# mims-harvard/ProCyon

Measured on AMD Instinct MI355X. Metric: phenotype-gen tokens/sec (ProCyon-Full greedy generation, end to end), higher is better.
Workload: dtype bf16; 1 GPU; configs[1]: ProCyon-Full (ESM2-650M + Llama-3-8B geometry=full) bf16 batch=1, 1024-residue protein, 512-token prompt, 256-token greedy generation; parallelism=single GPU

## Files before the change

include/pcy.h:

```cpp
#ifndef PCY_H
#define PCY_H
#include <stddef.h>
#include <stdint.h>

#ifdef __cplusplus
extern "C" {
#endif

#define PCY_ABI_VERSION 13

typedef struct pcy_ctx pcy_ctx;

enum { PCY_EPI_STORE = 0, PCY_EPI_RESID = 1, PCY_EPI_GELU_ERF = 2, PCY_EPI_GELU_ESM = 3, PCY_EPI_SWIGLU = 4 };
enum { PCY_POOL_MEAN = 0, PCY_POOL_MEAN_CORRECTED = 1, PCY_POOL_MAX = 2 };

int pcy_abi_version(void);
unsigned long long pcy_debug_dispatch_count(int kind);
unsigned long long pcy_debug_extend_grouped_count(void);
const char* pcy_last_error(void);
int pcy_ctx_create(int device_id, void* stream, pcy_ctx** out);
void pcy_ctx_destroy(pcy_ctx* ctx);
int pcy_ctx_sync(pcy_ctx* ctx);
int pcy_timer_start(pcy_ctx* ctx);
int pcy_timer_stop(pcy_ctx* ctx, float* ms_out);
// ... 169 lines not shown
  const int32_t* forced;
  int32_t* counters;
  int32_t* last;
  int32_t cap, W;
  int32_t ngram_max, ngram_min;
} pcy_look_state;
int pcy_look_draft(pcy_ctx*, const pcy_llama_desc*, const pcy_look_state*, const pcy_gen_state*, void* embeds_out);
int pcy_look_verify(pcy_ctx*, const pcy_llama_desc*, const pcy_look_state*, const pcy_gen_state*, const void* logits);
unsigned long long pcy_debug_look_count(int which);
int pcy_attn_window(pcy_ctx*, void* qkv, int ld, const pcy_kv_cache* kv, int layer, void* o, int ldo, const int32_t* pos, const void* cos_t,
                    const void* sin_t, int W, int H, int Hkv, int dh);
int pcy_attn_window_chunk(void);
int pcy_llama_decode_window(pcy_ctx*, const pcy_llama_desc*, const pcy_kv_cache*, const pcy_gen_state*, const void* embeds, int W,
                            void* logits_out);
unsigned long long pcy_debug_decode_window_count(void);
int pcy_llama_greedy(pcy_ctx*, const pcy_llama_desc*, const pcy_kv_cache*, const pcy_gen_state*, int B, int n_steps,
                     int use_graph);
int pcy_sample_pick(pcy_ctx*, const pcy_llama_desc*, const pcy_kv_cache*, const pcy_gen_state*, int B, int advance_pos,
                    float temperature, float nucleus_prob, const float* uniforms, void* probs_out);
int pcy_llama_sample(pcy_ctx*, const pcy_llama_desc*, const pcy_kv_cache*, const pcy_gen_state*, int B, int n_steps,
                     float temperature, float nucleus_prob, const float* uniforms);
typedef struct {
  int32_t* out; int32_t max_len;
  float* cur; float* cur_new;
  int32_t* next_tok;
  int32_t* src;
  int32_t* anc;
  uint8_t* has_eos;
  int32_t* blk_eos; int32_t* ticket;
  int32_t* pos; int32_t* step; int32_t* done;
// ... 40 lines not shown
```

procyon_amd/_lib.py:

```python
from __future__ import annotations

import ctypes as C
import os

_HERE = os.path.dirname(os.path.abspath(__file__))
LIB_PATH = os.environ.get("PCY_LIB") or os.path.join(_HERE, "libpcy.so")

EPI_STORE, EPI_RESID, EPI_GELU_ERF, EPI_GELU_ESM, EPI_SWIGLU = range(5)
POOL_MEAN, POOL_MEAN_CORRECTED, POOL_MAX = range(3)
ABI_VERSION = 13
(DISPATCH_GEMM_128, DISPATCH_GEMM_64, DISPATCH_GEMM_BIG, DISPATCH_GEMM_BIG_PERSIST, DISPATCH_GEMM_SPLITK, DISPATCH_GEMM_FP8, DISPATCH_ATTN_FAST,
 DISPATCH_DEC_STEP_GQA, DISPATCH_GEMM_MID, DISPATCH_ESM_GRAPH, DISPATCH_DEC_STEP_MHA, DISPATCH_DEC_LAYER, DISPATCH_DEC_STEP_NB, DISPATCH_DEC_STEP_MB,
 DISPATCH_DEC_LOOP_STREAM, DISPATCH_DEC_LOOP_MFMA, DISPATCH_SHARED_PREFIX, DISPATCH_XENT, DISPATCH_EXTEND,
 DISPATCH_EXTEND_PACKED) = range(20)
DISPATCH_DECODE = dict(step_gqa=DISPATCH_DEC_STEP_GQA, step_mha=DISPATCH_DEC_STEP_MHA, layer=DISPATCH_DEC_LAYER, step_nb=DISPATCH_DEC_STEP_NB,
                       step_mb=DISPATCH_DEC_STEP_MB, loop_stream=DISPATCH_DEC_LOOP_STREAM, loop_mfma=DISPATCH_DEC_LOOP_MFMA)
ATTN_ROUTE_DH32, ATTN_ROUTE_DH64, ATTN_ROUTE_LDS128_1, ATTN_ROUTE_LDS128_2 = range(4)

vp = C.c_void_p
i32 = C.c_int32
ci = C.c_int


class MlpDesc(C.Structure):
# ... 119 lines not shown
    "pcy_attn_decode_shared": (ci, [vp, vp, ci, C.POINTER(KvCache), ci, vp, ci, vp, vp, vp, vp, ci, ci, ci, ci]),
    "pcy_llama_decode_gemm_mq": (ci, [vp, C.POINTER(LlamaDesc), C.POINTER(KvCache), C.POINTER(GenState), ci]),
    "pcy_debug_attn_mq_count": (C.c_ulonglong, []),
    "pcy_gemv_w8": (ci, [vp, vp, vp, vp, ci, vp, vp, ci, vp, C.c_float, ci, ci, ci, ci, ci]),
    "pcy_llama_decode_w8": (ci, [vp, C.POINTER(LlamaDesc), C.POINTER(LlamaLayerFp8), C.POINTER(KvCache), C.POINTER(GenState), ci]),
    "pcy_llama_greedy_w8": (ci, [vp, C.POINTER(LlamaDesc), C.POINTER(LlamaLayerFp8), C.POINTER(KvCache), C.POINTER(GenState), ci, ci, ci]),
    "pcy_debug_decode_w8_count": (C.c_ulonglong, []),
    "pcy_greedy_pick": (ci, [vp, C.POINTER(LlamaDesc), C.POINTER(KvCache), C.POINTER(GenState), ci, ci]),
    "pcy_look_draft": (ci, [vp, C.POINTER(LlamaDesc), C.POINTER(LookState), C.POINTER(GenState), vp]),
    "pcy_look_verify": (ci, [vp, C.POINTER(LlamaDesc), C.POINTER(LookState), C.POINTER(GenState), vp]),
    "pcy_debug_look_count": (C.c_ulonglong, [ci]),
    "pcy_attn_window": (ci, [vp, vp, ci, C.POINTER(KvCache), ci, vp, ci, vp, vp, vp, ci, ci, ci, ci]),
    "pcy_attn_window_chunk": (ci, []),
    "pcy_llama_decode_window": (ci, [vp, C.POINTER(LlamaDesc), C.POINTER(KvCache), C.POINTER(GenState), vp, ci, vp]),
    "pcy_debug_decode_window_count": (C.c_ulonglong, []),
    "pcy_llama_greedy": (ci, [vp, C.POINTER(LlamaDesc), C.POINTER(KvCache), C.POINTER(GenState), ci, ci, ci]),
    "pcy_sample_pick": (ci, [vp, C.POINTER(LlamaDesc), C.POINTER(KvCache), C.POINTER(GenState), ci, ci, C.c_float, C.c_float, vp, vp]),
    "pcy_llama_sample": (ci, [vp, C.POINTER(LlamaDesc), C.POINTER(KvCache), C.POINTER(GenState), ci, ci, C.c_float, C.c_float, vp]),
    "pcy_beam_step": (ci, [vp, vp, ci, ci, ci, ci, C.c_float, C.POINTER(BeamState)]),
    "pcy_kv_reorder": (ci, [vp, C.POINTER(LlamaDesc), C.POINTER(KvCache), vp, ci, ci]),
    "pcy_kv_reorder_range": (ci, [vp, C.POINTER(LlamaDesc), C.POINTER(KvCache), vp, ci, ci, ci]),
    "pcy_llama_beam_steps": (ci, [vp, C.POINTER(LlamaDesc), C.POINTER(KvCache), C.POINTER(GenState), ci, ci, ci, C.c_float, C.POINTER(BeamState), vp, ci, ci]),
}

_lib = None


class PcyError(RuntimeError):
    pass

# ... 25 lines not shown
```

procyon_amd/csrc/pcy_elem.hip:

```cpp
#include "pcy_internal.h"
#include "pcy_pick.h"

namespace {

constexpr int NT = 256;

__global__ __launch_bounds__(NT) void rmsnorm_kernel(const bf16_t* __restrict__ x, const bf16_t* __restrict__ w,
                                                     bf16_t* __restrict__ y, int d, float eps, int cast) {
  __shared__ float red[NT / 64];
  const bf16_t* xr = x + (size_t)blockIdx.x * d;
  bf16_t* yr = y + (size_t)blockIdx.x * d;
  float ss = 0.f;
  for (int k = threadIdx.x * 8; k < d; k += NT * 8) {
    const uint4 v = *reinterpret_cast<const uint4*>(xr + k);
    const uint32_t u[4] = {v.x, v.y, v.z, v.w};
#pragma unroll
    for (int j = 0; j < 4; ++j) { float a = lo_bf(u[j]), b = hi_bf(u[j]); ss += a * a + b * b; }
  }
  ss = block_sum<NT>(ss, red);
  const float rstd = rsqrtf(ss / (float)d + eps);
  for (int k = threadIdx.x * 8; k < d; k += NT * 8) {
    const uint4 v = *reinterpret_cast<const uint4*>(xr + k);
    const uint4 g = *reinterpret_cast<const uint4*>(w + k);
    const uint32_t u[4] = {v.x, v.y, v.z, v.w}, gg[4] = {g.x, g.y, g.z, g.w};
// ... 375 lines not shown
  const int w = threadIdx.x >> 6;
  if ((threadIdx.x & 63) == 0) { redv[w] = best; redi[w] = bi; }
  __syncthreads();
  best = redv[0]; bi = redi[0];
  for (int i = 1; i < PICK_NT / 64; ++i)
    if (redv[i] > best || (redv[i] == best && redi[i] < bi)) { best = redv[i]; bi = redi[i]; }
  float se = 0.f;
  for (int i = lo + threadIdx.x; i < hi; i += PICK_NT) se += expf(bf2f(lg[i]) - best);
  se = block_sum<PICK_NT>(se, red);
  if (threadIdx.x == 0) part[b * PICK_NB + c] = PickPartial{best, bi, best > -INFINITY ? se : 0.f, 0};
}

__global__ __launch_bounds__(256) void pick_stage2_kernel(const bf16_t* __restrict__ logits, int V, const PickPartial* __restrict__ part,
                                                          int32_t* __restrict__ next_tok, int32_t* __restrict__ tokens_out, int max_steps,
                                                          float* __restrict__ logprob, int32_t* __restrict__ step_dev, int32_t* __restrict__ pos_dev,
                                                          int advance_pos, int B) {
  const int l = threadIdx.x & 63;
  const int step = *step_dev;
  for (int b = threadIdx.x >> 6; b < B; b += 4) {
    float best, se;
    int bi;
    pick_merge_row(part[b * PICK_NB + l], best, bi, se);
    if (l == 0) {
      const float lsm = pick_logprob(logits + (size_t)b * V, bi, best, se);
      logprob[b] += lsm;
      next_tok[b] = bi;
      tokens_out[(size_t)b * max_steps + step] = bi;
    }
  }
  __syncthreads();
  if (threadIdx.x == 0) { if (advance_pos) *pos_dev += 1; *step_dev = step + 1; }
}

constexpr int SMP_NT = 1024;

__global__ __launch_bounds__(PICK_NT) void sample_stage1_kernel(const bf16_t* __restrict__ logits, int V, float temperature,
                                                                float4* __restrict__ part) {
  __shared__ float red[PICK_NT / 64];
  const int b = blockIdx.y, c = blockIdx.x;
  const int chunk = (V + PICK_NB - 1) / PICK_NB;
  const int lo = c * chunk, hi = (lo + chunk) < V ? (lo + chunk) : V;
  const bf16_t* lg = logits + (size_t)b * V;
  const bool scaled = temperature != 1.0f;
  float mr = -INFINITY, ms = -INFINITY;
  for (int i = lo + threadIdx.x; i < hi; i += PICK_NT) {
    const float v = bf2f(lg[i]);
// ... 852 lines not shown
  hipLaunchKernelGGL(transpose_v_kernel, dim3((maxpad + 63) / 64, nh * dh / 64, nseq), dim3(NT), 0, s, buf, ld, vcol0, dh, cu, vt_cu, vt, vt_total);
}
size_t pcy_pool_ws_bytes(int nprot, int d) { return (size_t)nprot * POOL_CH * d * 8; }
void pcy_launch_pool(hipStream_t s, const bf16_t* h, int d, const int32_t* seg, const int32_t* rng, int nprot, int mode, bf16_t* out,
                     void* ws) {
  if (nprot <= 0) return;
  float* wsum = reinterpret_cast<float*>(ws);
  int* wcnt = reinterpret_cast<int*>(wsum + (size_t)nprot * POOL_CH * d);
  hipLaunchKernelGGL(pool_partial_kernel, dim3(nprot, (d + 511) / 512, POOL_CH), dim3(NT), 0, s, h, d, seg, rng, mode, wsum, wcnt);
  hipLaunchKernelGGL(pool_finish_kernel, dim3(nprot, (d + NT - 1) / NT), dim3(NT), 0, s, wsum, wcnt, d, mode, out);
}
void pcy_launch_pick_stage1(hipStream_t s, const bf16_t* logits, int rows, int V, void* partials) {
  if (rows > 0) hipLaunchKernelGGL(pick_stage1_kernel, dim3(PICK_NB, rows), dim3(PICK_NT), 0, s, logits, V, reinterpret_cast<PickPartial*>(partials));
}
void pcy_launch_greedy_pick(hipStream_t s, const bf16_t* logits, int B, int V, int32_t* next_tok, int32_t* tokens_out,
                            int max_steps, float* logprob, int32_t* pos_dev, int32_t* step_dev, int advance_pos, void* partials) {
  hipLaunchKernelGGL(pick_stage1_kernel, dim3(PICK_NB, B), dim3(PICK_NT), 0, s, logits, V, reinterpret_cast<PickPartial*>(partials));
  hipLaunchKernelGGL(pick_stage2_kernel, dim3(1), dim3(256), 0, s, logits, V, reinterpret_cast<const PickPartial*>(partials), next_tok,
                     tokens_out, max_steps, logprob, step_dev, pos_dev, advance_pos, B);
}
int pcy_sample_max_vocab() { return SMP_NT * SMP_KMAX; }
void pcy_launch_sample_step(hipStream_t s, const bf16_t* logits, int B, int V, float temperature, float nucleus_p, const float* uniforms,
                            unsigned* hist, bf16_t* probs_out, int32_t* next_tok, int32_t* tokens_out, int max_steps, float* logprob,
                            int32_t* pos_dev, int32_t* step_dev, int advance_pos, void* partials, bf16_t* pbits) {
  hipLaunchKernelGGL(sample_stage1_kernel, dim3(PICK_NB, B), dim3(PICK_NT), 0, s, logits, V, temperature, reinterpret_cast<float4*>(partials));
  hipLaunchKernelGGL(sample_probs_kernel, dim3(PICK_NB, B), dim3(PICK_NT), 0, s, logits, V, reinterpret_cast<const float4*>(partials), temperature,
                     nucleus_p > 0.f ? 1 : 0, hist, pbits);
  hipLaunchKernelGGL(sample_stage2_kernel, dim3(B), dim3(SMP_NT), 0, s, logits, V, reinterpret_cast<const float4*>(partials), temperature,
                     nucleus_p, uniforms, hist, probs_out, next_tok, tokens_out, max_steps, logprob, step_dev, B, pbits);
  hipLaunchKernelGGL(sample_advance_kernel, dim3(1), dim3(64), 0, s, pos_dev, step_dev, advance_pos);
}
void pcy_launch_copy_rows(hipStream_t s, const bf16_t* src, int lds_, bf16_t* dst, int ldd, const int32_t* rows, int nrows, int d) {
  if (nrows > 0) hipLaunchKernelGGL(copy_rows_kernel, dim3(nrows), dim3(NT), 0, s, src, lds_, dst, ldd, rows, d);
}
// ... 39 lines not shown
```

procyon_amd/csrc/pcy_engine.hip:

```cpp
#include <stdio.h>
#include <stdlib.h>
#include <stdarg.h>
#include <string.h>
#include <dlfcn.h>
#include <vector>

#include "../../include/pcy.h"
#include "pcy_internal.h"

namespace {

thread_local char g_err[512] = "";

int fail(int code, const char* fmt, ...) {
  va_list ap;
  va_start(ap, fmt);
  vsnprintf(g_err, sizeof(g_err), fmt, ap);
  va_end(ap);
  return code;
}

#define HIP_TRY(expr)                                                                       \
  do {                                                                                      \
    hipError_t e_ = (expr);                                                                 \
    if (e_ != hipSuccess) return fail(2, "%s failed: %s (%s:%d)", #expr, hipGetErrorString(e_), __FILE__, __LINE__); \
  } while (0)

inline size_t align_up(size_t v, size_t a) { return (v + a - 1) / a * a; }

inline bool kv_shared(const pcy_kv_cache* kv) { return kv->prefix_k != nullptr || kv->prefix_v != nullptr || kv->prefix_T != 0; }
inline int kv_cap(const pcy_kv_cache* kv) { return kv->Tmax + (kv_shared(kv) ? kv->prefix_T : 0); }
unsigned long long g_pcy_extend_grouped = 0;
unsigned long long g_pcy_look[2] = {0, 0};
unsigned long long g_pcy_decode_gemm = 0;
unsigned long long g_pcy_attn_mq = 0;
unsigned long long g_pcy_decode_w8 = 0;
unsigned long long g_pcy_decode_window = 0;

}

void pcy_set_error(const char* fmt, ...) {
  va_list ap;
  va_start(ap, fmt);
  vsnprintf(g_err, sizeof(g_err), fmt, ap);
  va_end(ap);
}

struct DecodeGraphKey {
  int kind;
  int B;
  PcySwitches sw;
  const void *model, *layers, *embed, *kv_k, *kv_v, *pos, *step, *next_tok, *logits, *keep;
// ... 368 lines not shown
  const pcy_llama_desc* m = cx.m;
  PcyGemvArgs g{};
  g.W = (const bf16_t*)W; g.x = in; g.y = out; g.N = N; g.K = K; g.B = cx.B; g.ldx = K; g.ldy = N; g.epi = epi;
  g.force_stream = p.nb_on; g.krot = krot;
  if (splitk) { g.splitk_ws = cx.sk_ws; g.splitk_ws_bytes = cx.sk_bytes; }
  if (epi == EPI_RESID) {
    g.resid = out;
    if (p.batched && cx.B <= 32) { g.next_rms_w = (const bf16_t*)ln; g.next_xn = cx.xn; g.fused_next = xn_ready; g.rms_eps = m->rms_eps; g.rms_cast = m->rms_cast; }
  } else {
    g.rms_eps = m->rms_eps; g.rms_cast = m->rms_cast;
    if (p.batched) g.x = cx.xn; else g.rms_w = (const bf16_t*)ln;
  }
  return g;
}

void enqueue_decode(pcy_ctx* c, const pcy_llama_desc* m, const pcy_kv_cache* kv, const pcy_gen_state* st, int B, const PcySwitches& sw, bool layers_only = false) {
  hipStream_t s = c->stream;
  const int d = m->d, H = m->n_heads, dh = m->head_dim, F = m->ffn;
  const DecodeCx cx = decode_cx(c, m, kv, st, B);
  const DecodePlan p = plan_decode(c, m, kv, B, sw);
  if (layers_only) {
    if (p.epoch_word) pcy_launch_bump(s, p.epoch_word);
    if (p.tag_word) pcy_launch_bump(s, p.tag_word);
  } else {
    pcy_launch_embed_tokens_dev(s, (const bf16_t*)m->embed, st->next_tok, cx.x, B, d, p.epoch_word, p.tag_word);
  }
  const size_t tag_stride = tag_words_per_layer(m);
  bool step_done = false;
  bool try_layer = p.path == DEC_STEP_GQA || p.path == DEC_STEP_MHA || p.path == DEC_LAYERS;
  int xn_ready = 0;
  if (p.path == DEC_STEP_NB) {
    const PcyDecodeStepArgs sa = step_args(cx, c->nb_tags[B], pcy_decode_nb_tag_words(B), 2 * AO_FLAGS, pcy_decode_nb_line_words(B));
    step_done = pcy_launch_decode_step_nb(s, c->device, attn_args(cx, p, -1), block_args(cx, p.tag_word, mc_trace(sw)), mlp_args(cx, p.tag_word), sa, c->n_cu,
                                          c->ao_sync, B, sw.nb_ub);
    if (step_done) ++g_pcy_dispatch[PCY_DISPATCH_DEC_STEP_NB];
  } else if (p.path == DEC_STEP_GQA || p.path == DEC_STEP_MHA) {
    const PcyDecodeStepArgs sa = step_args(cx, c->mc_tags, tag_stride, AO_FLAGS, 32 * 256);
    step_done = pcy_launch_decode_step(s, attn_args(cx, p, -1), block_args(cx, p.tag_word, mc_trace(sw)), mlp_args(cx, p.tag_word), sa, c->n_cu,
                                       c->ao_sync);
// ... 41 lines not shown
    pcy_launch_gemv(s, proj_args(cx, p, L.wgu, L.ln2, cx.x, d, cx.act, F, EPI_SWIGLU, false, p.krot, nullptr));
    const PcyGemvArgs w = proj_args(cx, p, L.wdown, l + 1 < m->n_layers ? m->layers[l + 1].ln1 : m->final_norm, cx.act, F, cx.x, d, EPI_RESID, true, 0, &xn_ready);
    if (p.nb_on && pcy_launch_gemv_kwin4(s, w)) continue;
    pcy_launch_gemv(s, w);
  }
  if (layers_only) return;
  PcyGemvArgs h{};
  h.W = (const bf16_t*)m->lm_head; h.x = cx.x; h.y = (bf16_t*)st->logits; h.rms_w = (const bf16_t*)m->final_norm; h.rms_eps = m->rms_eps;
  h.rms_cast = m->rms_cast; h.N = m->vocab; h.K = d; h.B = B; h.ldx = d; h.ldy = m->vocab; h.epi = EPI_STORE;
  if (p.batched_head && !(p.nb_on && B <= 4)) {
    if (!xn_ready) pcy_launch_rmsnorm(s, cx.x, (const bf16_t*)m->final_norm, cx.xn, B, d, m->rms_eps, m->rms_cast);
    h.x = cx.xn; h.rms_w = nullptr;
  } else if (p.nb_on) {
    h.force_stream = 1;
  }
  pcy_launch_gemv(s, h);
}

__global__ void store_logits_kernel(const bf16_t* __restrict__ logits, bf16_t* __restrict__ all, const int32_t* step_dev,
                                    int B, int V, int ld) {
  const size_t step = (size_t)(*step_dev);
  const int chunks = (V + 7) / 8;
  const bool vec = (ld % 8 == 0) && ((reinterpret_cast<uintptr_t>(all) & 15) == 0);
  for (size_t i = (size_t)blockIdx.x * blockDim.x + threadIdx.x; i < (size_t)B * chunks; i += (size_t)gridDim.x * blockDim.x) {
    const int b = (int)(i / chunks), c = (int)(i % chunks);
    const bf16_t* src = logits + (size_t)b * V + c * 8;
    bf16_t* dst = all + (step * B + b) * ld + c * 8;
    if (vec && c * 8 + 8 <= V) {
      const uint32_t w0 = src[0] | ((uint32_t)src[1] << 16), w1 = src[2] | ((uint32_t)src[3] << 16);
      const uint32_t w2 = src[4] | ((uint32_t)src[5] << 16), w3 = src[6] | ((uint32_t)src[7] << 16);
      *reinterpret_cast<uint4*>(dst) = make_uint4(w0, w1, w2, w3);
    } else {
      for (int e = 0; e < 8 && c * 8 + e < V; ++e) dst[e] = src[e];
    }
  }
}
void enqueue_store_logits(hipStream_t s, const void* logits, void* all, int ld, const int32_t* step_dev, int B, int V) {
  if (all) hipLaunchKernelGGL(store_logits_kernel, dim3(B >= 8 ? 256 : 64), dim3(256), 0, s, (const bf16_t*)logits, (bf16_t*)all, step_dev, B, V, ld > 0 ? ld : V);
}
void enqueue_pick(pcy_ctx* c, const pcy_llama_desc* m, const pcy_gen_state* st, int B, int advance_pos, int Tmax) {
  enqueue_store_logits(c->stream, st->logits, st->logits_all, st->logits_all_ld, st->step, B, m->vocab);
  pcy_launch_greedy_pick(c->stream, (const bf16_t*)st->logits, B, m->vocab, st->next_tok, st->tokens_out, st->max_steps,
                         st->logprob, st->pos, st->step, advance_pos, carve_decode_ws(c->ws, m, B, Tmax).partials);
}

void enqueue_sample(pcy_ctx* c, const pcy_llama_desc* m, const pcy_gen_state* st, int B, int advance_pos, int Tmax, float temperature,
                    float nucleus_p, const float* uniforms, bf16_t* probs_out) {
  hipStream_t s = c->stream;
  if (nucleus_p > 0.f) temperature = 1.0f;
  enqueue_store_logits(s, st->logits, st->logits_all, st->logits_all_ld, st->step, B, m->vocab);
  void* partials = carve_decode_ws(c->ws, m, B, Tmax).partials;
  pcy_launch_sample_step(s, (const bf16_t*)st->logits, B, m->vocab, temperature, nucleus_p, uniforms, c->smp_hist, probs_out, st->next_tok,
                         st->tokens_out, st->max_steps, st->logprob, st->pos, st->step, advance_pos, partials, c->smp_pbits);
}
int ensure_sample_state(pcy_ctx* c, int B, int V) {
  if ((size_t)B * V > c->smp_pbits_elems) {
    if (c->smp_pbits) { HIP_TRY(hipStreamSynchronize(c->stream)); HIP_TRY(hipFree(c->smp_pbits)); c->smp_pbits = nullptr; c->smp_pbits_elems = 0; }
    HIP_TRY(hipMalloc(reinterpret_cast<void**>(&c->smp_pbits), (size_t)B * V * 2));
    c->smp_pbits_elems = (size_t)B * V;
  }
  if (B <= c->smp_hist_rows) return 0;
  if (c->smp_hist) { HIP_TRY(hipStreamSynchronize(c->stream)); HIP_TRY(hipFree(c->smp_hist)); c->smp_hist = nullptr; }
  HIP_TRY(hipMalloc(reinterpret_cast<void**>(&c->smp_hist), (size_t)B * 65536 * sizeof(unsigned)));
  HIP_TRY(hipMemset(c->smp_hist, 0, (size_t)B * 65536 * sizeof(unsigned)));
  c->smp_hist_rows = B;
// ... 901 lines not shown
      e0 = hipStreamEndCapture(c->cap_stream, &g);
    }
    c->stream = user;
    if (e0 != hipSuccess) return fail(2, "%s graph capture failed: %s", what, hipGetErrorString(e0));
    HIP_TRY(hipGraphInstantiate(&c->graph, g, nullptr, nullptr, 0));
    hipGraphDestroy(g);
    memcpy(&c->graph_key, &key, sizeof(key));
  }
  for (int i = 0; i < n_steps; ++i) HIP_TRY(hipGraphLaunch(c->graph, c->stream));
  return 0;
}
int replay_decode_graph(pcy_ctx* c, const pcy_llama_desc* m, const pcy_kv_cache* kv, const pcy_gen_state* st, int B, int n_steps, int kind, const PcySwitches& sw) {
  DecodeGraphKey key;
  decode_graph_key(key, c, m, kv, st, B, kind, sw);
  key.tokens_out = st->tokens_out; key.logprob = st->logprob; key.logits_all = st->logits_all; key.logits_all_ld = st->logits_all_ld; key.max_steps = st->max_steps;
  return replay_graph(c, key, n_steps, "decode-step", [&] {
    enqueue_decode(c, m, kv, st, B, sw);
    if (kind == 0) enqueue_pick(c, m, st, B, 1, kv_cap(kv));
  });
}
}
extern "C" {
int pcy_llama_prefill(pcy_ctx* c, const pcy_llama_desc* m, const pcy_kv_cache* kv, const void* embeds, const uint8_t* keep,
                      const int32_t* pos, const int32_t* cu, const int32_t* vt_cu, int B, int T, const int32_t* logit_rows,
                      int n_logit_rows, void* logits_out, void* hidden_out, const int32_t* sum_rows, int n_sum_rows,
                      void* hidden_sum_out) {
  PrefillReq r{};
  r.embeds = embeds; r.keep = keep; r.pos = pos; r.cu = cu; r.vt_cu = vt_cu; r.B = B; r.T = T; r.logit_rows = logit_rows; r.n_logit_rows = n_logit_rows;
  r.logits_out = logits_out; r.hidden_out = hidden_out; r.sum_rows = sum_rows; r.n_sum_rows = n_sum_rows; r.hidden_sum_out = hidden_sum_out;
  return llama_prefill_impl(c, m, kv, r);
}
int pcy_llama_prefill_all(pcy_ctx* c, const pcy_llama_desc* m, const pcy_kv_cache* kv, const void* embeds, const uint8_t* keep,
                          const int32_t* pos, const int32_t* cu, const int32_t* vt_cu, int B, int T, const int32_t* logit_rows,
// ... 110 lines not shown
  ++g_pcy_look[1];
  return check_launch("pcy_look_verify");
}
unsigned long long pcy_debug_look_count(int which) { return (which == 0 || which == 1) ? g_pcy_look[which] : 0; }


int pcy_llama_greedy(pcy_ctx* c, const pcy_llama_desc* m, const pcy_kv_cache* kv, const pcy_gen_state* st, int B, int n_steps,
                     int use_graph) {
  PCY_STICKY(c);
  if (B > kv->B) return fail(1, "pcy_llama_greedy: B=%d exceeds cache rows %d", B, kv->B);
  if (int r = c->reserve(decode_ws_bytes(m, B, kv_cap(kv)))) return r;
  const PcySwitches sw = pcy_read_switches();
  if (int r = ensure_decode_state(c, m, B, sw)) return r;
  if (int r = check_decode_cache(c, m, kv, B, sw, "pcy_llama_greedy")) return r;
  if (!use_graph) {
    for (int i = 0; i < n_steps; ++i) {
      enqueue_decode(c, m, kv, st, B, sw);
      enqueue_pick(c, m, st, B, 1, kv_cap(kv));
    }
    return check_launch("pcy_llama_greedy");
  }
  return replay_decode_graph(c, m, kv, st, B, n_steps, 0, sw);
}

int pcy_llama_decode_graph(pcy_ctx* c, const pcy_llama_desc* m, const pcy_kv_cache* kv, const pcy_gen_state* st, int B) {
  PCY_STICKY(c);
  if (B > kv->B) return fail(1, "pcy_llama_decode_graph: B=%d exceeds cache rows %d", B, kv->B);
  if (int r = c->reserve(decode_ws_bytes(m, B, kv_cap(kv)))) return r;
  const PcySwitches sw = pcy_read_switches();
  if (int r = ensure_decode_state(c, m, B, sw)) return r;
  if (int r = check_decode_cache(c, m, kv, B, sw, "pcy_llama_decode_graph")) return r;
  return replay_decode_graph(c, m, kv, st, B, 1, 1, sw);
}

// ... 257 lines not shown
  PCY_STICKY(c);
  const char* what = "pcy_llama_decode_window";
  if (!m || !kv || !st || !kv->k || !kv->v || !st->pos || !m->layers || !embeds || !logits_out) return fail(1, "%s: model, cache, state, embeds or logits_out incomplete", what);
  if (st->keep) return fail(1, "%s: a keep mask is not supported (lookahead prompts are unpadded)", what);
  if (m->layers_fp8) return fail(1, "%s: fp8 projections are not supported on this step", what);
  const int d = m->d, H = m->n_heads, Hkv = m->n_kv_heads, dh = m->head_dim, F = m->ffn;
  if (int r = check_win_call(kv, W, H, Hkv, dh, what)) return r;
  if (d % 16 || F % 16 || (H * dh) % 16 || ((H + 2 * Hkv) * dh) % 16) return fail(1, "%s: d, ffn, H*dh, (H+2Hkv)*dh must be multiples of 16", what);
  const size_t need = align_up(decode_ws_bytes(m, W, kv_cap(kv)), 256) + win_ws_bytes(pcy_attn_win_plan(W, H, Hkv, dh, kv->Tmax));
  if (int r = c->reserve(need)) return r;
  HIP_TRY(hipMemcpyAsync(carve_decode_ws(c->ws, m, W, kv_cap(kv)).x, embeds, (size_t)W * d * 2, hipMemcpyDeviceToDevice, c->stream));
  enqueue_decode_window(c, m, kv, st, W, logits_out);
  return check_launch(what);
}
unsigned long long pcy_debug_decode_window_count(void) { return g_pcy_decode_window; }
int pcy_attn_window_chunk(void) { return pcy_attn_win_chunk(); }

int pcy_attn_window(pcy_ctx* c, void* qkv, int ld, const pcy_kv_cache* kv, int layer, void* o, int ldo, const int32_t* pos, const void* cos_t,
                    const void* sin_t, int W, int H, int Hkv, int dh) {
  PCY_STICKY(c);
  const char* what = "pcy_attn_window";
  if (!qkv || !kv || !kv->k || !kv->v || !o || !pos || !cos_t || !sin_t || layer < 0) return fail(1, "%s: qkv, cache, o, pos or rope tables missing (layer=%d)", what, layer);
  if (int r = check_win_call(kv, W, H, Hkv, dh, what)) return r;
  if (ld % 8 || ld < (H + 2 * Hkv) * dh || ldo % 8 || ldo < H * dh) return fail(1, "%s: ld=%d ldo=%d (rows must be 16-byte aligned and hold all heads)", what, ld, ldo);
  if (int r = c->reserve(win_ws_bytes(pcy_attn_win_plan(W, H, Hkv, dh, kv->Tmax)))) return r;
  if (!pcy_launch_attn_window(c->stream, win_attn_args((const bf16_t*)qkv, ld, kv, layer, (bf16_t*)o, ldo, pos, (const bf16_t*)cos_t, (const bf16_t*)sin_t,
                                                       W, H, Hkv, dh, c->ws)))
    return fail(1, "%s: shape not covered", what);
  return check_launch(what);
}
// ... 25 lines not shown
  return check_launch("pcy_sample_pick");
}

int pcy_llama_sample(pcy_ctx* c, const pcy_llama_desc* m, const pcy_kv_cache* kv, const pcy_gen_state* st, int B, int n_steps,
                     float temperature, float nucleus_prob, const float* uniforms) {
  PCY_STICKY(c);
  if (B > kv->B) return fail(1, "pcy_llama_sample: B=%d exceeds cache rows %d", B, kv->B);
  if (!(temperature > 0.f) || nucleus_prob >= 1.f) return fail(1, "pcy_llama_sample: temperature > 0 and nucleus_prob < 1 required");
  if (m->vocab > pcy_sample_max_vocab()) return fail(1, "pcy_llama_sample: vocabulary %d unsupported (<= %d)", m->vocab, pcy_sample_max_vocab());
  if (int r = c->reserve(decode_ws_bytes(m, B, kv_cap(kv)))) return r;
  const PcySwitches sw = pcy_read_switches();
  if (int r = ensure_decode_state(c, m, B, sw)) return r;
  if (int r = check_decode_cache(c, m, kv, B, sw, "pcy_llama_sample")) return r;
  if (int r = ensure_sample_state(c, B, m->vocab)) return r;
  for (int i = 0; i < n_steps; ++i) {
    enqueue_decode(c, m, kv, st, B, sw);
    enqueue_sample(c, m, st, B, 1, kv_cap(kv), temperature, nucleus_prob, uniforms, nullptr);
  }
  return check_launch("pcy_llama_sample");
}

int pcy_beam_step(pcy_ctx* c, const void* logits, int vocab, int B, int beam, int group_size, float diversity_penalty,
                  const pcy_beam_state* st) {
  PCY_STICKY(c);
  if (B <= 0 || beam <= 0 || beam > 32 || group_size <= 0 || beam % group_size)
    return fail(1, "pcy_beam_step: beam=%d (1..32) must be a multiple of group_size=%d", beam, group_size);
  if (vocab <= 0 || vocab > 163840) return fail(1, "pcy_beam_step: vocab %d unsupported (<= 163840)", vocab);
  if (int r = ensure_beam_ws(c, B, beam)) return r;
  pcy_launch_beam_step(c->stream, (const bf16_t*)logits, vocab, B, beam, group_size, diversity_penalty, beam_state_args(st), c->beam_ws);
  return check_launch("pcy_beam_step");
}

// ... 79 lines not shown
```

procyon_amd/csrc/pcy_gemv.hip:

```cpp
#include <stdlib.h>
#include "pcy_internal.h"
#include "pcy_handover.h"
#include "pcy_mlp_chain.h"

namespace {

#ifndef PCY_GEMV_DIRECTX
#define PCY_GEMV_DIRECTX 0
#endif
constexpr int GEMV_THREADS = 256;
constexpr int GEMV_WAVES = 4;
constexpr int XS_BYTES_MAX = 65536;

template <int NB, int EPI, bool RMS, int UN>
__global__ __launch_bounds__(GEMV_THREADS) void gemv_kernel(PcyGemvArgs a, int KC) {
  constexpr int RW = (EPI == EPI_SWIGLU) ? 8 : 4;
  extern __shared__ __attribute__((aligned(16))) char smem[];
  bf16_t* xs = reinterpret_cast<bf16_t*>(smem);
  float* red = reinterpret_cast<float*>(smem + (size_t)NB * KC * 2);
  const int lane = threadIdx.x & 63, wave = threadIdx.x >> 6;
  const int K = a.K;

  int rows[RW];
  bool rvalid[RW];
// ... 136 lines not shown
template <int NB, int EPI, bool RMS, int R>
__global__ __launch_bounds__(512) void gemv_stream_kernel(PcyGemvArgs a, int units) {
  constexpr bool DIRECTX = PCY_GEMV_DIRECTX && !RMS;
  constexpr int RW = (EPI == EPI_SWIGLU) ? 2 * R : R;
  constexpr int UN = 16 / RW;
  extern __shared__ __attribute__((aligned(16))) char smem[];
  bf16_t* xs = reinterpret_cast<bf16_t*>(smem);
  float* red = reinterpret_cast<float*>(smem + (size_t)NB * a.K * 2);
  const int lane = threadIdx.x & 63, wave = threadIdx.x >> 6;
  const int K = a.K;
  const int nit = (K + 511) >> 9;
  const int wpb = blockDim.x >> 6;
  const int nw = gridDim.x * wpb;
  const int nthr = blockDim.x;
  const int nrows = (EPI == EPI_SWIGLU) ? 2 * a.N : a.N;

  auto row_off = [&](int u, int i) -> size_t {
    int r;
    if (EPI == EPI_SWIGLU) {
      const int f = u * R + (i % R);
      const int fc = f < a.N ? f : a.N - 1;
      r = (fc >> 4) * 32 + (fc & 15) + (i >= R ? 16 : 0);
    } else {
      r = u * R + i;
      r = r < nrows ? r : nrows - 1;
    }
    return (size_t)r * K;
  };
  const bool krot = a.krot && (K & 511) == 0;
  auto rot = [&](int u, int it) { if (!krot) return it; const int r = it + ((u * R) >> 2) % nit; return r >= nit ? r - nit : r; };
// ... 41 lines not shown
        const int n = u * R + i;
        if (n >= a.N) continue;
#pragma unroll
        for (int b = 0; b < NB; ++b) {
          float v;
          if (EPI == EPI_SWIGLU) {
            const float g = rbf(acc[i][b]), up = rbf(acc[i + R][b]);
            v = rbf(silu_f(g)) * up;
          } else {
            v = rbf(acc[i][b] + (a.bias ? bf2f(a.bias[n]) : 0.f));
            if (EPI == EPI_RESID) v = rbf(v + bf2f(a.resid[(size_t)b * a.ldy + n]));
            if (EPI == EPI_GELU_ERF) v = rbf(gelu_erf_f(v));
            if (EPI == EPI_GELU_ESM) v = gelu_esm_chain(v);
          }
          a.y[(size_t)b * a.ldy + n] = f2bf(v);
        }
      }
    }
    zero_acc();
  };

  uint4 wa[UN][RW], wb[UN][RW];
  int u = blockIdx.x * wpb + wave;
  int it0 = 0;
  bool have = u < units;
  auto next_pos = [&](int cu, int cit, int& nu_, int& nit_) {
    nit_ = cit + UN; nu_ = cu;
    if (nit_ >= nit) { nit_ = 0; nu_ = cu + nw; }
  };

  constexpr int MAXX = RMS ? 4 : 8;
  const bool xfirst = NB == 1 && !DIRECTX && K <= MAXX * nthr * 8 && a.plain_loads != 2;
// ... 136 lines not shown
    for (int w = 4; w <= 8; ++w) {
      const int waves = bl * w;
      if (waves > GEMV_MAX_WAVES) continue;
      const int per = (units + waves - 1) / waves;
      const double cost = (double)per * waves / units + 1e-3 * (GEMV_MAX_WAVES - waves) / GEMV_MAX_WAVES;
      if (cost < best) { best = cost; blocks = bl; wpb = w; }
    }
  if (units < GEMV_CUS * 4) { blocks = (units + 3) / 4; wpb = 4; }
}

template <int NB, int EPI, bool RMS, int R>
void launch_stream(hipStream_t s, const PcyGemvArgs& a) {
  const int units = (a.N + R - 1) / R;
  int blocks, wpb;
  pick_grid(units, blocks, wpb);
  const size_t smem = (size_t)NB * a.K * 2 + 64;
  hipLaunchKernelGGL((gemv_stream_kernel<NB, EPI, RMS, R>), dim3(blocks), dim3(wpb * 64), smem, s, a, units);
}

template <int NB, int EPI, bool RMS>
void launch_nb(hipStream_t s, const PcyGemvArgs& a) {
  if ((size_t)NB * a.K * 2 <= XS_BYTES_MAX) {
    if ((a.N + 3) / 4 < GEMV_MAX_WAVES) launch_stream<NB, EPI, RMS, 2>(s, a);
    else launch_stream<NB, EPI, RMS, 4>(s, a);
    return;
  }
  int KC = a.K;
  if ((size_t)NB * KC * 2 > XS_BYTES_MAX) KC = (XS_BYTES_MAX / (NB * 2)) & ~511;
  const size_t smem = (size_t)NB * KC * 2 + 64;
  const int blocks = (a.N + 15) / 16;
  constexpr int UN = (EPI == EPI_SWIGLU) ? 2 : 4;
  hipLaunchKernelGGL((gemv_kernel<NB, EPI, RMS, UN>), dim3(blocks), dim3(GEMV_THREADS), smem, s, a, KC);
// ... 625 lines not shown
  return true;
}


int pcy_mfma_min_batch() { return 4; }

bool pcy_launch_gemv_kwin4(hipStream_t s, const PcyGemvArgs& a) {
  if (a.K % 2048 || a.bias || a.rms_w || (a.epi != EPI_RESID && a.epi != EPI_STORE)) return false;
  hipLaunchKernelGGL(gemv_kwin4_kernel, dim3((a.N + 3) / 4), dim3(256), 0, s, a);
  return true;
}

void pcy_launch_gemv(hipStream_t s, const PcyGemvArgs& a00) {
  PcyGemvArgs a0 = a00;
  a0.plain_loads = 0;
  if (!a0.force_stream && (a0.B >= pcy_mfma_min_batch() || a0.force_mfma) && a0.K % 128 == 0 && a0.rms_w == nullptr && (a0.ldx % 8) == 0) {
    if (a0.B > 32) {
      if (a0.defer_finish) *a0.defer_finish = 0;
      a0.defer_finish = nullptr;
      a0.next_rms_w = nullptr; a0.next_xn = nullptr; a0.fused_next = nullptr;
    }
    for (int b0 = 0; b0 < a0.B; b0 += 32) {
      PcyGemvArgs a = a0;
      a.B = (a0.B - b0) < 32 ? (a0.B - b0) : 32;
      a.x = a0.x + (size_t)b0 * a0.ldx;
      a.y = a0.y + (size_t)b0 * a0.ldy;
      if (a0.resid) a.resid = a0.resid + (size_t)b0 * a0.ldy;
      switch (a.epi) {
        case EPI_STORE: launch_mfma<EPI_STORE>(s, a); break;
        case EPI_RESID: launch_mfma<EPI_RESID>(s, a); break;
// ... 23 lines not shown
```

procyon_amd/csrc/pcy_internal.h:

```cpp
#pragma once
#include "pcy_common.h"
#include "pcy_switch.h"

struct PcyGemvArgs {
  const bf16_t* W;
  const bf16_t* x;
  bf16_t* y;
  const bf16_t* bias;
  const bf16_t* resid;
  const bf16_t* rms_w;
  float rms_eps;
  int rms_cast;
  int N, K, B, ldx, ldy, epi;
  int plain_loads;
  float* splitk_ws; size_t splitk_ws_bytes;
  const bf16_t* next_rms_w; bf16_t* next_xn; int* fused_next;
  int* defer_finish;
  int force_stream;
  int force_mfma;
  int krot;
};
void pcy_launch_gemv(hipStream_t s, const PcyGemvArgs& a);

struct PcyGemvW8Args {
  const uint8_t* W;
  const float* scale;
  const bf16_t* x;
  bf16_t* y;
  const bf16_t* resid;
  const bf16_t* rms_w;
  float rms_eps;
  int rms_cast;
  int N, K, B, ldx, ldy, epi;
};
int pcy_gemv_w8_rows_per_pass(int K);
// ... 252 lines not shown
  int B, Tmax; float scale, rms_eps; int rms_cast;
  unsigned* flags;
  const unsigned* epoch;
  unsigned* err;
  unsigned long long* trace;
  int abl;
};
size_t pcy_decode_mb_flag_words();
int pcy_decode_mb_ds(int B);
bool pcy_decode_mb_fits(int B, int Tmax);
bool pcy_launch_decode_step_mb(hipStream_t s, int device, const PcyMbArgs& a, int n_cu);

size_t pcy_pool_ws_bytes(int nprot, int d);
void pcy_launch_pool(hipStream_t s, const bf16_t* h, int d, const int32_t* seg, const int32_t* rng, int nprot,
                     int mode, bf16_t* out, void* ws);
void pcy_launch_greedy_pick(hipStream_t s, const bf16_t* logits, int B, int V, int32_t* next_tok, int32_t* tokens_out,
                            int max_steps, float* logprob, int32_t* pos_dev, int32_t* step_dev, int advance_pos,
                            void* partials );
void pcy_launch_pick_stage1(hipStream_t s, const bf16_t* logits, int rows, int V, void* partials);
struct PcyLookArgs {
  int32_t* hist; int32_t* n_hist; int32_t* window; const int32_t* forced; int32_t* counters; int32_t* last;
  int cap, W, gmax, gmin;
  int32_t* pos; int32_t* step; int32_t* next_tok; int32_t* tokens_out; float* logprob; int max_steps;
};
size_t pcy_look_verify_ws_bytes(int W);
void pcy_launch_look_draft(hipStream_t s, const PcyLookArgs& a, const bf16_t* embed, int V, int d, bf16_t* embeds_out );
void pcy_launch_look_verify(hipStream_t s, const PcyLookArgs& a, const bf16_t* logits , int V, bf16_t* logits_all, int logits_all_ld,
                            void* partials );
void pcy_launch_retrieval_dot_f32(hipStream_t s, const float* query, int Q, const void* targets, int targets_bf16, int N, int D, float eps, float* sims);
size_t pcy_retrieval_dot_smem(int D);
void pcy_launch_retrieval_rank_f32(hipStream_t s, const float* sims, int Q, int N, int k, int32_t* idx_out, float* score_out);
int pcy_sample_max_vocab();
void pcy_launch_sample_step(hipStream_t s, const bf16_t* logits, int B, int V, float temperature, float nucleus_p, const float* uniforms,
// ... 24 lines not shown
```

procyon_amd/csrc/pcy_switch.h:

```cpp
#pragma once
#include <stdint.h>
#include <stdlib.h>
#include <string.h>
#include <type_traits>

#define PCY_SWITCH_NAMES(X)                                                                                                                \
  X(attn_o) X(mlp_chain) X(decode_layer) X(decode_step) X(attn_qkv_finish) X(finish_norm) X(fp8_fused_norm) X(prefill_post_qkv) X(gemv_lds) \
  X(gemv_mfma4) X(fa_vrow) X(gelu_fast) X(esm_graph) X(lds_prefetch) X(decode_nb) X(decode_nb_step) X(beam_graph) X(kv_permute)             \
  X(decode_mb_step) X(beam_prefill_once) X(beam_kv_suffix) X(beam_kv_shared)
enum PcySwitch {
#define X(n) PCY_SW_##n,
  PCY_SWITCH_NAMES(X)
#undef X
  PCY_SW_COUNT
};
static_assert(PCY_SW_COUNT <= 32, "PcySwitches::off_mask holds one bit per name");

inline bool pcy_list_has(const char* list, const char* name) {
  if (!list) return false;
  const size_t n = strlen(name);
  for (const char* p = list; (p = strstr(p, name)) != nullptr; p += n)
    if ((p == list || p[-1] == ',') && (p[n] == 0 || p[n] == ',')) return true;
  return false;
}
// ... 39 lines not shown
```

Measured before the change: 394.8 tokens/s.

## Fuse logits recording into LM-head GEMV and next-token embedding into greedy pick

Removes two kernel launches per greedy decode step. The LM-head streaming GEMV now writes the logits row into the logits_all history itself, staging values in shared memory with per-round atomic counters, so the separate store_logits kernel is skipped. The pick stage-2 kernel also gathers the next token's embedding row into the decode input buffer and bumps the epoch/tag words, so the next step skips its embed kernel; the first step's embedding is issued once before the loop or graph. This adds extra shared memory and atomics to the GEMV and couples step boundaries, which matters for graph replay correctness.

```diff
diff --git a/include/pcy.h b/include/pcy.h
--- a/include/pcy.h
+++ b/include/pcy.h
@@ -207,6 +207,7 @@
 int pcy_llama_decode_window(pcy_ctx*, const pcy_llama_desc*, const pcy_kv_cache*, const pcy_gen_state*, const void* embeds, int W,
                             void* logits_out);
 unsigned long long pcy_debug_decode_window_count(void);
+unsigned long long pcy_debug_step_seam_count(int which);
 int pcy_llama_greedy(pcy_ctx*, const pcy_llama_desc*, const pcy_kv_cache*, const pcy_gen_state*, int B, int n_steps,
                      int use_graph);
 int pcy_sample_pick(pcy_ctx*, const pcy_llama_desc*, const pcy_kv_cache*, const pcy_gen_state*, int B, int advance_pos,
diff --git a/procyon_amd/_lib.py b/procyon_amd/_lib.py
--- a/procyon_amd/_lib.py
+++ b/procyon_amd/_lib.py
@@ -157,6 +157,7 @@
     "pcy_attn_window_chunk": (ci, []),
     "pcy_llama_decode_window": (ci, [vp, C.POINTER(LlamaDesc), C.POINTER(KvCache), C.POINTER(GenState), vp, ci, vp]),
     "pcy_debug_decode_window_count": (C.c_ulonglong, []),
+    "pcy_debug_step_seam_count": (C.c_ulonglong, [ci]),
     "pcy_llama_greedy": (ci, [vp, C.POINTER(LlamaDesc), C.POINTER(KvCache), C.POINTER(GenState), ci, ci, ci]),
     "pcy_sample_pick": (ci, [vp, C.POINTER(LlamaDesc), C.POINTER(KvCache), C.POINTER(GenState), ci, ci, C.c_float, C.c_float, vp, vp]),
     "pcy_llama_sample": (ci, [vp, C.POINTER(LlamaDesc), C.POINTER(KvCache), C.POINTER(GenState), ci, ci, C.c_float, C.c_float, vp]),
diff --git a/procyon_amd/csrc/pcy_elem.hip b/procyon_amd/csrc/pcy_elem.hip
--- a/procyon_amd/csrc/pcy_elem.hip
+++ b/procyon_amd/csrc/pcy_elem.hip
@@ -413,7 +413,8 @@
 __global__ __launch_bounds__(256) void pick_stage2_kernel(const bf16_t* __restrict__ logits, int V, const PickPartial* __restrict__ part,
                                                           int32_t* __restrict__ next_tok, int32_t* __restrict__ tokens_out, int max_steps,
                                                           float* __restrict__ logprob, int32_t* __restrict__ step_dev, int32_t* __restrict__ pos_dev,
-                                                          int advance_pos, int B) {
+                                                          int advance_pos, int B, PcyPickHandover ho) {
+  __shared__ int tok_s[PICK_HANDOVER_MAX_ROWS];
   const int l = threadIdx.x & 63;
   const int step = *step_dev;
   for (int b = threadIdx.x >> 6; b < B; b += 4) {
@@ -425,10 +426,22 @@
       logprob[b] += lsm;
       next_tok[b] = bi;
       tokens_out[(size_t)b * max_steps + step] = bi;
+      if (ho.x && b < PICK_HANDOVER_MAX_ROWS) tok_s[b] = bi;
     }
   }
   __syncthreads();
   if (threadIdx.x == 0) { if (advance_pos) *pos_dev += 1; *step_dev = step + 1; }
+  if (ho.x) {
+    if (threadIdx.x == 0) {
+      if (ho.epoch) *ho.epoch += 1;
+      if (ho.epoch2) *ho.epoch2 += 1;
+    }
+    const int per = ho.d / 8;
+    for (int i = threadIdx.x; i < B * per; i += 256) {
+      const int b = i / per, k = (i - b * per) * 8;
+      *reinterpret_cast<uint4*>(ho.x + (size_t)b * ho.d + k) = *reinterpret_cast<const uint4*>(ho.table + (size_t)tok_s[b] * ho.d + k);
+    }
+  }
 }
 
 constexpr int SMP_NT = 1024;
@@ -1311,10 +1324,13 @@
   if (rows > 0) hipLaunchKernelGGL(pick_stage1_kernel, dim3(PICK_NB, rows), dim3(PICK_NT), 0, s, logits, V, reinterpret_cast<PickPartial*>(partials));
 }
 void pcy_launch_greedy_pick(hipStream_t s, const bf16_t* logits, int B, int V, int32_t* next_tok, int32_t* tokens_out,
-                            int max_steps, float* logprob, int32_t* pos_dev, int32_t* step_dev, int advance_pos, void* partials) {
+                            int max_steps, float* logprob, int32_t* pos_dev, int32_t* step_dev, int advance_pos, void* partials,
+                            const PcyPickHandover* handover) {
+  PcyPickHandover ho{};
+  if (handover && B <= PICK_HANDOVER_MAX_ROWS && handover->d % 8 == 0) ho = *handover;
   hipLaunchKernelGGL(pick_stage1_kernel, dim3(PICK_NB, B), dim3(PICK_NT), 0, s, logits, V, reinterpret_cast<PickPartial*>(partials));
   hipLaunchKernelGGL(pick_stage2_kernel, dim3(1), dim3(256), 0, s, logits, V, reinterpret_cast<const PickPartial*>(partials), next_tok,
-                     tokens_out, max_steps, logprob, step_dev, pos_dev, advance_pos, B);
+                     tokens_out, max_steps, logprob, step_dev, pos_dev, advance_pos, B, ho);
 }
 int pcy_sample_max_vocab() { return SMP_NT * SMP_KMAX; }
 void pcy_launch_sample_step(hipStream_t s, const bf16_t* logits, int B, int V, float temperature, float nucleus_p, const float* uniforms,
diff --git a/procyon_amd/csrc/pcy_engine.hip b/procyon_amd/csrc/pcy_engine.hip
--- a/procyon_amd/csrc/pcy_engine.hip
+++ b/procyon_amd/csrc/pcy_engine.hip
@@ -36,6 +36,7 @@
 unsigned long long g_pcy_attn_mq = 0;
 unsigned long long g_pcy_decode_w8 = 0;
 unsigned long long g_pcy_decode_window = 0;
+unsigned long long g_pcy_seam[3] = {0, 0, 0};
 
 }
 
@@ -434,7 +435,9 @@
   return g;
 }
 
-void enqueue_decode(pcy_ctx* c, const pcy_llama_desc* m, const pcy_kv_cache* kv, const pcy_gen_state* st, int B, const PcySwitches& sw, bool layers_only = false) {
+struct SeamPlan { bool embed_done; int* rec_done; };
+void enqueue_decode(pcy_ctx* c, const pcy_llama_desc* m, const pcy_kv_cache* kv, const pcy_gen_state* st, int B, const PcySwitches& sw, bool layers_only = false,
+                    const SeamPlan* seam = nullptr) {
   hipStream_t s = c->stream;
   const int d = m->d, H = m->n_heads, dh = m->head_dim, F = m->ffn;
   const DecodeCx cx = decode_cx(c, m, kv, st, B);
@@ -442,7 +445,7 @@
   if (layers_only) {
     if (p.epoch_word) pcy_launch_bump(s, p.epoch_word);
     if (p.tag_word) pcy_launch_bump(s, p.tag_word);
-  } else {
+  } else if (!(seam && seam->embed_done)) {
     pcy_launch_embed_tokens_dev(s, (const bf16_t*)m->embed, st->next_tok, cx.x, B, d, p.epoch_word, p.tag_word);
   }
   const size_t tag_stride = tag_words_per_layer(m);
@@ -514,7 +517,11 @@
   } else if (p.nb_on) {
     h.force_stream = 1;
   }
+  if (seam && seam->rec_done && st->logits_all && B == 1) {
+    h.rec = (bf16_t*)st->logits_all; h.rec_ld = st->logits_all_ld > 0 ? st->logits_all_ld : m->vocab; h.rec_step = st->step; h.rec_done = seam->rec_done;
+  }
   pcy_launch_gemv(s, h);
+  if (h.rec_done && *h.rec_done) ++g_pcy_seam[0];
 }
 
 __global__ void store_logits_kernel(const bf16_t* __restrict__ logits, bf16_t* __restrict__ all, const int32_t* step_dev,
@@ -536,19 +543,43 @@
   }
 }
 void enqueue_store_logits(hipStream_t s, const void* logits, void* all, int ld, const int32_t* step_dev, int B, int V) {
+  if (all) ++g_pcy_seam[1];
   if (all) hipLaunchKernelGGL(store_logits_kernel, dim3(B >= 8 ? 256 : 64), dim3(256), 0, s, (const bf16_t*)logits, (bf16_t*)all, step_dev, B, V, ld > 0 ? ld : V);
 }
-void enqueue_pick(pcy_ctx* c, const pcy_llama_desc* m, const pcy_gen_state* st, int B, int advance_pos, int Tmax) {
-  enqueue_store_logits(c->stream, st->logits, st->logits_all, st->logits_all_ld, st->step, B, m->vocab);
+void enqueue_pick(pcy_ctx* c, const pcy_llama_desc* m, const pcy_gen_state* st, int B, int advance_pos, int Tmax, bool recorded = false,
+                  const PcyPickHandover* handover = nullptr) {
+  if (!recorded) enqueue_store_logits(c->stream, st->logits, st->logits_all, st->logits_all_ld, st->step, B, m->vocab);
+  if (handover) ++g_pcy_seam[2];
   pcy_launch_greedy_pick(c->stream, (const bf16_t*)st->logits, B, m->vocab, st->next_tok, st->tokens_out, st->max_steps,
-                         st->logprob, st->pos, st->step, advance_pos, carve_decode_ws(c->ws, m, B, Tmax).partials);
+                         st->logprob, st->pos, st->step, advance_pos, carve_decode_ws(c->ws, m, B, Tmax).partials, handover);
+}
+bool seam_hands_over(const pcy_llama_desc* m, int B, const PcySwitches& sw) {
+  return !sw.off(PCY_SW_step_seam) && B <= PICK_HANDOVER_MAX_ROWS && m->d % 8 == 0;
+}
+void enqueue_seam_embed(pcy_ctx* c, const pcy_llama_desc* m, const pcy_kv_cache* kv, const pcy_gen_state* st, int B, const PcySwitches& sw) {
+  const DecodePlan p = plan_decode(c, m, kv, B, sw);
+  pcy_launch_embed_tokens_dev(c->stream, (const bf16_t*)m->embed, st->next_tok, decode_cx(c, m, kv, st, B).x, B, m->d, p.epoch_word, p.tag_word);
+}
+void enqueue_greedy_step(pcy_ctx* c, const pcy_llama_desc* m, const pcy_kv_cache* kv, const pcy_gen_state* st, int B, const PcySwitches& sw) {
+  if (sw.off(PCY_SW_step_seam)) {
+    enqueue_decode(c, m, kv, st, B, sw);
+    enqueue_pick(c, m, st, B, 1, kv_cap(kv));
+    return;
+  }
+  int recorded = 0;
+  const bool hand = seam_hands_over(m, B, sw);
+  const SeamPlan seam{hand, &recorded};
+  enqueue_decode(c, m, kv, st, B, sw, false, &seam);
+  const DecodePlan p = plan_decode(c, m, kv, B, sw);
+  const PcyPickHandover ho{(const bf16_t*)m->embed, decode_cx(c, m, kv, st, B).x, m->d, p.epoch_word, p.tag_word};
+  enqueue_pick(c, m, st, B, 1, kv_cap(kv), recorded != 0, hand ? &ho : nullptr);
 }
 
 void enqueue_sample(pcy_ctx* c, const pcy_llama_desc* m, const pcy_gen_state* st, int B, int advance_pos, int Tmax, float temperature,
-                    float nucleus_p, const float* uniforms, bf16_t* probs_out) {
+                    float nucleus_p, const float* uniforms, bf16_t* probs_out, bool recorded = false) {
   hipStream_t s = c->stream;
   if (nucleus_p > 0.f) temperature = 1.0f;
-  enqueue_store_logits(s, st->logits, st->logits_all, st->logits_all_ld, st->step, B, m->vocab);
+  if (!recorded) enqueue_store_logits(s, st->logits, st->logits_all, st->logits_all_ld, st->step, B, m->vocab);
   void* partials = carve_decode_ws(c->ws, m, B, Tmax).partials;
   pcy_launch_sample_step(s, (const bf16_t*)st->logits, B, m->vocab, temperature, nucleus_p, uniforms, c->smp_hist, probs_out, st->next_tok,
                          st->tokens_out, st->max_steps, st->logprob, st->pos, st->step, advance_pos, partials, c->smp_pbits);
@@ -1480,9 +1511,10 @@
   DecodeGraphKey key;
   decode_graph_key(key, c, m, kv, st, B, kind, sw);
   key.tokens_out = st->tokens_out; key.logprob = st->logprob; key.logits_all = st->logits_all; key.logits_all_ld = st->logits_all_ld; key.max_steps = st->max_steps;
+  if (kind == 0 && n_steps > 0 && seam_hands_over(m, B, sw)) enqueue_seam_embed(c, m, kv, st, B, sw);
   return replay_graph(c, key, n_steps, "decode-step", [&] {
-    enqueue_decode(c, m, kv, st, B, sw);
-    if (kind == 0) enqueue_pick(c, m, st, B, 1, kv_cap(kv));
+    if (kind == 0) enqueue_greedy_step(c, m, kv, st, B, sw);
+    else enqueue_decode(c, m, kv, st, B, sw);
   });
 }
 }
@@ -1623,10 +1655,8 @@
   if (int r = ensure_decode_state(c, m, B, sw)) return r;
   if (int r = check_decode_cache(c, m, kv, B, sw, "pcy_llama_greedy")) return r;
   if (!use_graph) {
-    for (int i = 0; i < n_steps; ++i) {
-      enqueue_decode(c, m, kv, st, B, sw);
-      enqueue_pick(c, m, st, B, 1, kv_cap(kv));
-    }
+    if (n_steps > 0 && seam_hands_over(m, B, sw)) enqueue_seam_embed(c, m, kv, st, B, sw);
+    for (int i = 0; i < n_steps; ++i) enqueue_greedy_step(c, m, kv, st, B, sw);
     return check_launch("pcy_llama_greedy");
   }
   return replay_decode_graph(c, m, kv, st, B, n_steps, 0, sw);
@@ -1914,6 +1944,7 @@
   return check_launch(what);
 }
 unsigned long long pcy_debug_decode_window_count(void) { return g_pcy_decode_window; }
+unsigned long long pcy_debug_step_seam_count(int which) { return (which >= 0 && which < 3) ? g_pcy_seam[which] : 0; }
 int pcy_attn_window_chunk(void) { return pcy_attn_win_chunk(); }
 
 int pcy_attn_window(pcy_ctx* c, void* qkv, int ld, const pcy_kv_cache* kv, int layer, void* o, int ldo, const int32_t* pos, const void* cos_t,
@@ -1969,8 +2000,10 @@
   if (int r = check_decode_cache(c, m, kv, B, sw, "pcy_llama_sample")) return r;
   if (int r = ensure_sample_state(c, B, m->vocab)) return r;
   for (int i = 0; i < n_steps; ++i) {
-    enqueue_decode(c, m, kv, st, B, sw);
-    enqueue_sample(c, m, st, B, 1, kv_cap(kv), temperature, nucleus_prob, uniforms, nullptr);
+    int recorded = 0;
+    const SeamPlan seam{false, &recorded};
+    enqueue_decode(c, m, kv, st, B, sw, false, sw.off(PCY_SW_step_seam) ? nullptr : &seam);
+    enqueue_sample(c, m, st, B, 1, kv_cap(kv), temperature, nucleus_prob, uniforms, nullptr, recorded != 0);
   }
   return check_launch("pcy_llama_sample");
 }
diff --git a/procyon_amd/csrc/pcy_gemv.hip b/procyon_amd/csrc/pcy_gemv.hip
--- a/procyon_amd/csrc/pcy_gemv.hip
+++ b/procyon_amd/csrc/pcy_gemv.hip
@@ -174,6 +174,15 @@
   const int nw = gridDim.x * wpb;
   const int nthr = blockDim.x;
   const int nrows = (EPI == EPI_SWIGLU) ? 2 * a.N : a.N;
+  constexpr bool REC = NB == 1 && EPI == EPI_STORE && RMS;
+  bf16_t* rstage = reinterpret_cast<bf16_t*>(smem + (size_t)NB * a.K * 2 + 64);
+  int* rcnt = reinterpret_cast<int*>(rstage + (size_t)((units + nw - 1) / nw) * 32);
+  bf16_t* rec_row = nullptr;
+  int rnd = 0;
+  if (REC && a.rec) {
+    rec_row = a.rec + (size_t)(*a.rec_step) * a.rec_ld;
+    for (int i = threadIdx.x; i < (units + nw - 1) / nw; i += nthr) rcnt[i] = 0;
+  }
 
   auto row_off = [&](int u, int i) -> size_t {
     int r;
@@ -245,8 +254,28 @@
             if (EPI == EPI_GELU_ESM) v = gelu_esm_chain(v);
           }
           a.y[(size_t)b * a.ldy + n] = f2bf(v);
+          if (REC && rec_row) rstage[rnd * 32 + wave * R + i] = f2bf(v);
         }
       }
+    }
+    if (REC && rec_row) {
+      const int ub = u - wave;
+      int last = 0;
+      if (lane == 0) {
+        const int waves_in = units - ub < wpb ? units - ub : wpb;
+        last = __hip_atomic_fetch_add(&rcnt[rnd], 1, __ATOMIC_ACQ_REL, __HIP_MEMORY_SCOPE_WORKGROUP) == waves_in - 1;
+      }
+      if (__builtin_amdgcn_readfirstlane(last)) {
+        const int n0 = ub * R, cnt = a.N - n0 < wpb * R ? a.N - n0 : wpb * R;
+        bf16_t* dst = rec_row + n0;
+        const bf16_t* src = rstage + rnd * 32;
+        if (cnt == wpb * R && (cnt & 7) == 0 && (reinterpret_cast<uintptr_t>(dst) & 15) == 0) {
+          if (lane < cnt / 8) reinterpret_cast<uint4*>(dst)[lane] = reinterpret_cast<const uint4*>(src)[lane];
+        } else if (lane < cnt) {
+          dst[lane] = src[lane];
+        }
+      }
+      ++rnd;
     }
     zero_acc();
   };
@@ -413,8 +442,16 @@
   const int units = (a.N + R - 1) / R;
   int blocks, wpb;
   pick_grid(units, blocks, wpb);
-  const size_t smem = (size_t)NB * a.K * 2 + 64;
-  hipLaunchKernelGGL((gemv_stream_kernel<NB, EPI, RMS, R>), dim3(blocks), dim3(wpb * 64), smem, s, a, units);
+  size_t smem = (size_t)NB * a.K * 2 + 64;
+  PcyGemvArgs k = a;
+  if (NB == 1 && EPI == EPI_STORE && RMS && a.rec && a.rec_step) {
+    smem += (size_t)((units + blocks * wpb - 1) / (blocks * wpb)) * (32 * 2 + 4);
+    if (a.rec_ld <= 0) k.rec_ld = a.N;
+    if (a.rec_done) *a.rec_done = 1;
+  } else {
+    k.rec = nullptr;
+  }
+  hipLaunchKernelGGL((gemv_stream_kernel<NB, EPI, RMS, R>), dim3(blocks), dim3(wpb * 64), smem, s, k, units);
 }
 
 template <int NB, int EPI, bool RMS>
@@ -1070,6 +1107,8 @@
 void pcy_launch_gemv(hipStream_t s, const PcyGemvArgs& a00) {
   PcyGemvArgs a0 = a00;
   a0.plain_loads = 0;
+  if (a0.rec_done) *a0.rec_done = 0;
+  if (a0.B != 1) a0.rec = nullptr;
   if (!a0.force_stream && (a0.B >= pcy_mfma_min_batch() || a0.force_mfma) && a0.K % 128 == 0 && a0.rms_w == nullptr && (a0.ldx % 8) == 0) {
     if (a0.B > 32) {
       if (a0.defer_finish) *a0.defer_finish = 0;
diff --git a/procyon_amd/csrc/pcy_internal.h b/procyon_amd/csrc/pcy_internal.h
--- a/procyon_amd/csrc/pcy_internal.h
+++ b/procyon_amd/csrc/pcy_internal.h
@@ -19,6 +19,7 @@
   int force_stream;
   int force_mfma;
   int krot;
+  bf16_t* rec; int rec_ld; const int32_t* rec_step; int* rec_done;
 };
 void pcy_launch_gemv(hipStream_t s, const PcyGemvArgs& a);
 
@@ -301,9 +302,11 @@
 size_t pcy_pool_ws_bytes(int nprot, int d);
 void pcy_launch_pool(hipStream_t s, const bf16_t* h, int d, const int32_t* seg, const int32_t* rng, int nprot,
                      int mode, bf16_t* out, void* ws);
+constexpr int PICK_HANDOVER_MAX_ROWS = 8;
+struct PcyPickHandover { const bf16_t* table; bf16_t* x; int d; unsigned* epoch; unsigned* epoch2; };
 void pcy_launch_greedy_pick(hipStream_t s, const bf16_t* logits, int B, int V, int32_t* next_tok, int32_t* tokens_out,
                             int max_steps, float* logprob, int32_t* pos_dev, int32_t* step_dev, int advance_pos,
-                            void* partials );
+                            void* partials , const PcyPickHandover* handover = nullptr);
 void pcy_launch_pick_stage1(hipStream_t s, const bf16_t* logits, int rows, int V, void* partials);
 struct PcyLookArgs {
   int32_t* hist; int32_t* n_hist; int32_t* window; const int32_t* forced; int32_t* counters; int32_t* last;
diff --git a/procyon_amd/csrc/pcy_switch.h b/procyon_amd/csrc/pcy_switch.h
--- a/procyon_amd/csrc/pcy_switch.h
+++ b/procyon_amd/csrc/pcy_switch.h
@@ -7,7 +7,7 @@
 #define PCY_SWITCH_NAMES(X)                                                                                                                \
   X(attn_o) X(mlp_chain) X(decode_layer) X(decode_step) X(attn_qkv_finish) X(finish_norm) X(fp8_fused_norm) X(prefill_post_qkv) X(gemv_lds) \
   X(gemv_mfma4) X(fa_vrow) X(gelu_fast) X(esm_graph) X(lds_prefetch) X(decode_nb) X(decode_nb_step) X(beam_graph) X(kv_permute)             \
-  X(decode_mb_step) X(beam_prefill_once) X(beam_kv_suffix) X(beam_kv_shared)
+  X(decode_mb_step) X(beam_prefill_once) X(beam_kv_suffix) X(beam_kv_shared) X(step_seam)
 enum PcySwitch {
 #define X(n) PCY_SW_##n,
   PCY_SWITCH_NAMES(X)
```

After: 395.3 tokens/s, median of 5. About the same (+0.1%).
